# HiLab-git/FPL-plus

Hardware: NVIDIA B200
Metric: train_voxels_per_s (higher is better)
Workload: dtype bf16

## Files before the change

### fpl-plus_b200/build.py

```python
import os
import shutil
import subprocess
import sys

HERE = os.path.dirname(os.path.abspath(__file__))
CSRC = os.path.join(HERE, "csrc")
LIB = os.path.join(HERE, "libfplplus_b200.so")
SOURCES = ["api.cu", "dsbn.cu", "loss.cu", "filter.cu", "conv_direct.cu", "conv_tc.cu", "conv_wgrad_tc.cu", "conv_wgrad_hs.cu", "convt_tc.cu", "conv_tc_dfold.cu", "grad.cu", "adam.cu", "datapath.cu", "head.cu", "head_tc.cu", "stem_tc.cu", "upsample.cu"]
NVCC_FLAGS = ["-gencode", "arch=compute_100a,code=sm_100a", "-lineinfo", "-O3", "-std=c++17",
              "-Xcompiler", "-fPIC", "--use_fast_math=false"]


def _nvcc():
    for cand in (os.environ.get("NVCC"), shutil.which("nvcc"), "/usr/local/cuda/bin/nvcc"):
        if cand and os.path.exists(cand):
            return cand
    raise RuntimeError("nvcc not found; the fplplus_b200 CUDA library cannot be built")


def needs_build():
    if not os.path.exists(LIB):
        return True
    t = os.path.getmtime(LIB)
    deps = [os.path.join(CSRC, f) for f in os.listdir(CSRC)] + [os.path.join(HERE, "..", "include", "fplplus_b200.h")]
# ... 37 lines not shown
```

### fpl-plus_b200/csrc/conv_tc_dfold.cu

```cuda
#include "common.cuh"
#include "tc_ptx.cuh"
#include "../../include/fplplus_b200.h"

namespace {

constexpr int kTileH = 16, kTileW = 8;
constexpr int kBoxH = kTileH + 2, kBoxW = kTileW + 2;
constexpr int kPlaneBytes = kBoxH * kBoxW * 16;
constexpr int kThreadsD = 192;
constexpr int kMaxStagesD = 8;
constexpr int kMaxDC = 16;

struct DfParams {
    const __nv_bfloat16* image;
    const float* bias;
    bf16x8* y;
    int y_c8tot, y_c8off;
    double* stats;
    int N, D, H, W, cin, cout;
    int x_c8tot, x_c8off;
    int nb, nslices, dc, ndc;
    int a_bytes, b_bytes, stages, tmem_cols;
    int pb;
    int tiles_h, tiles_w, total_items;
// ... 480 lines not shown
extern "C" int fpl_conv3d_dfold_prep_weight(const float* w, int cin, int cout, int transpose_flip, void* image, void* stream) {
    return dfold_prep(w, cin, cout, transpose_flip, 9, image, stream);
}

extern "C" int fpl_conv3d_k311_prep_weight(const float* w, int cin, int cout, void* image, void* stream) {
    return dfold_prep(w, cin, cout, 0, 1, image, stream);
}

namespace {
constexpr int kMaxDfBatch = 64;
struct DfPrepBatch {
    const float* w[kMaxDfBatch];
    __nv_bfloat16* image[kMaxDfBatch];
    int cin_eff[kMaxDfBatch], cout_eff[kMaxDfBatch], total[kMaxDfBatch];
    unsigned char tf[kMaxDfBatch], nb[kMaxDfBatch];
};
__global__ void dfold_prep_batch_kernel(const __grid_constant__ DfPrepBatch B) {
    FPL_PDL_WAIT();
    const int e = blockIdx.y;
    const float* __restrict__ w = B.w[e];
    __nv_bfloat16* image = B.image[e];
    const int cin_eff = B.cin_eff[e], cout_eff = B.cout_eff[e], nb = B.nb[e], tf = B.tf[e];
    const int ksteps = cin_eff / 16, n3 = 3 * nb;
    const int pairs = cin_eff * cout_eff;
    for (int r = blockIdx.x * blockDim.x + threadIdx.x; r < pairs; r += gridDim.x * blockDim.x) {
        const int el = r & 7, n = (r >> 3) % nb, jk = (r >> 3) / nb;
        const int in = jk * 8 + el, out = n;
        const float* src = tf ? w + ((int64_t)in * cout_eff + out) * 27 : w + ((int64_t)out * cin_eff + in) * 27;
#pragma unroll
        for (int jj = 0; jj < 3; ++jj) {
#pragma unroll
            for (int t9 = 0; t9 < 9; ++t9) {
                const int tap = (2 - jj) * 9 + t9;
                const float v = __ldg(src + (tf ? 26 - tap : tap));
                image[(((int64_t)t9 * ksteps * 2 + jk) * n3 + jj * nb + n) * 8 + el] = __float2bfloat16_rn(v);
            }
        }
    }
}
}

extern "C" int fpl_conv3d_dfold_prep_weight_batch(int count, const float* const* h_w, const int* h_cin, const int* h_cout,
                                                  const int* h_transpose_flip, void* const* h_images, void* stream) {
    FPL_REQUIRE(count >= 0 && count <= kMaxDfBatch, "fpl_conv3d_dfold_prep_weight_batch: count %d not in [0,%d]", count, kMaxDfBatch);
    if (count == 0) return 0;
    DfPrepBatch B;
    int max_total = 0;
    for (int e = 0; e < count; ++e) {
        const int tf = h_transpose_flip[e];
        const int cin_eff = tf ? h_cout[e] : h_cin[e], cout_eff = tf ? h_cin[e] : h_cout[e];
        DfCfg c;
        FPL_REQUIRE(make_df_cfg(cin_eff, cout_eff, 16, c), "fpl_conv3d_dfold_prep_weight_batch: unsupported channels (%d -> %d)", cin_eff, cout_eff);
        B.w[e] = h_w[e]; B.image[e] = (__nv_bfloat16*)h_images[e]; B.cin_eff[e] = cin_eff; B.cout_eff[e] = cout_eff;
        B.tf[e] = (unsigned char)tf; B.nb[e] = (unsigned char)c.nb; B.total[e] = c.nslices * c.b_bytes / 2;
        if (B.total[e] > max_total) max_total = B.total[e];
    }
    int bx = (max_total / 27 + 255) / 256;
    if (bx > 32) bx = 32;
    if (bx < 1) bx = 1;
    fpl_launch(dfold_prep_batch_kernel, dim3(bx, count), 256, 0, (cudaStream_t)stream, B);
    FPL_LAUNCH_CHECK();
    return 0;
}

static int dfold_launch(const void* x, int x_c8tot, int x_c8off, const void* image, const float* bias, void* y,
                        int y_c8tot, int y_c8off, double* stats, int n, int d, int h, int w, int cin, int cout, int taps,
                        int cin_a, void* stream, const EpiAct* act = nullptr, const EpiBwdRed* br = nullptr) {
    if (cin_a <= 0) cin_a = cin;
    DfCfg c;
    FPL_REQUIRE(make_df_cfg(cin, cout, d, c, taps, cin_a), "fpl_conv3d_tc_dfold: unsupported shape (%d -> %d, depth %d)", cin, cout, d);
    FPL_REQUIRE((reinterpret_cast<uintptr_t>(x) & 15) == 0 && (reinterpret_cast<uintptr_t>(image) & 15) == 0,
                "fpl_conv3d_tc_dfold: x/image must be 16-byte aligned");
    EncodeTiledFn encode = get_encode_fn();
    FPL_REQUIRE(encode != nullptr, "fpl_conv3d_tc_dfold: cuTensorMapEncodeTiled not available from the driver");
    CUtensorMap xmap;
    const int bw = (g_df_tma & 1) ? kTileW : kBoxW, bh = (g_df_tma & 8) ? kTileH : kBoxH;
    const int esz = (g_df_tma & 2) ? 8 : 2;
// ... 91 lines not shown
```

### fpl-plus_b200/lib.py

```python
import ctypes
import os
from ctypes import c_char_p, c_double, c_float, c_int, c_int64, c_longlong, c_uint64, c_void_p

from . import build as _build

_P = c_void_p
_I = c_int
_L = c_int64
_F = c_float
_U = c_uint64

_SIGNATURES = {
    "fpl_last_error": (c_char_p, []),
    "fpl_version": (_I, []),
    "fpl_set_sm_budget": (_I, [_I]),
    "fpl_launch_count": (c_longlong, [_I]),
    "fpl_device_is_sm100": (_I, []),
    "fpl_debug_set": (None, [_I, c_longlong]),
    "fpl_conv3d_weight_image_bytes": (_L, [_I, _I, _I]),
    "fpl_conv3d_prep_weight": (_I, [_P, _I, _I, _I, _I, _P, _P]),
    "fpl_conv3d_prep_weight_batch": (_I, [_I, ctypes.POINTER(c_void_p), ctypes.POINTER(_I), ctypes.POINTER(_I),
                                          ctypes.POINTER(_I), ctypes.POINTER(_I), ctypes.POINTER(c_void_p), _P]),
    "fpl_conv3d_tc": (_I, [_P, _I, _I, _P, _P, _P, _I, _I, _P] + [_I] * 7 + [_P]),
    "fpl_conv3d_dfold_image_bytes": (_L, [_I, _I]),
    "fpl_conv3d_dfold_prep_weight": (_I, [_P, _I, _I, _I, _P, _P]),
    "fpl_conv3d_dfold_prep_weight_batch": (_I, [_I, ctypes.POINTER(c_void_p), ctypes.POINTER(_I), ctypes.POINTER(_I),
                                                ctypes.POINTER(_I), ctypes.POINTER(c_void_p), _P]),
    "fpl_conv3d_tc_dfold": (_I, [_P, _I, _I, _P, _P, _P, _I, _I, _P] + [_I] * 6 + [_P]),
    "fpl_patch9_c8": (_I, [_P, _P, _I, _I, _I, _I, _I, _P]),
    "fpl_conv3d_k311_prep_weight": (_I, [_P, _I, _I, _P, _P]),
    "fpl_conv3d_tc_k311": (_I, [_P, _I, _I, _P, _P, _P, _I, _I, _P] + [_I] * 7 + [_P]),
    "fpl_conv3d_wgrad_tc_k311": (_I, [_P, _I, _I, _P, _I, _I, _P] + [_I] * 6 + [_P]),
    "fpl_conv3d_direct": (_I, [_P, _I, _I, _P, _P, _P, _I, _I, _P] + [_I] * 9 + [_P]),
    "fpl_conv3d_wgrad": (_I, [_P, _I, _I, _P, _I, _I, _P] + [_I] * 7 + [_P]),
    "fpl_conv3d_wgrad_tc": (_I, [_P, _I, _I, _P, _I, _I, _P] + [_I] * 7 + [_P]),
    "fpl_conv3d_wgrad_tc_tapmajor": (_I, [_P, _I, _I, _P, _I, _I, _P] + [_I] * 7 + [_P]),
    "fpl_wgrad_tapmajor_to_dw_batch": (_I, [_I, ctypes.POINTER(c_void_p), ctypes.POINTER(c_void_p), ctypes.POINTER(_I),
                                            ctypes.POINTER(_I), ctypes.POINTER(_I), ctypes.POINTER(_I), _P]),
    "fpl_dsbn_eval_affine_batch": (_I, [_I] + [ctypes.POINTER(c_void_p)] * 7 + [ctypes.POINTER(_I), _F, _P]),
    "fpl_conv3d_tc_act": (_I, [_P, _I, _I, _P, _P, _I, _I] + [_I] * 7 + [_P, _P, _P, _F, _U, _U, _P, _P]),
    "fpl_conv3d_tc_dfold_act": (_I, [_P, _I, _I, _P, _P, _I, _I] + [_I] * 6 + [_P, _P, _P, _P]),
    "fpl_conv3d_tc_k311_act": (_I, [_P, _I, _I, _P, _P, _I, _I] + [_I] * 7 + [_P, _P, _P, _P]),
    "fpl_maxpool_c8": (_I, [_P, _I, _I, _P, _I, _I, _I] + [_I] * 5 + [_P]),
    "fpl_head_fwd": (_I, [_P, _I, _I, _P, _P, _P] + [_I] * 6 + [_P]),
    "fpl_head_dgrad": (_I, [_P, _P, _P, _I, _I, _P, _I, _I, _P] + [_I] * 6 + [_P]),
    "fpl_upsample2x_c8": (_I, [_P, _I, _I, _P, _I, _I] + [_I] * 6 + [_P]),
    "fpl_upsample2x_c8_bwd": (_I, [_P, _I, _I, _P, _I, _I] + [_I] * 6 + [_P]),
    "fpl_channel_sum_c8": (_I, [_P, _I, _I, _P] + [_I] * 5 + [_P]),
    "fpl_grad_scatter_add": (_I, [_P, _P, _P, _I, _I, _P]),
    "fpl_stem_conv_fwd": (_I, [_P, _P, _P, _P, _I, _I, _P] + [_I] * 7 + [_P]),
    "fpl_stem_conv_wgrad": (_I, [_P, _P, _I, _I, _P] + [_I] * 7 + [_P]),
    "fpl_head_conv_fwd": (_I, [_P, _I, _I, _P, _P, _P] + [_I] * 6 + [_P]),
    "fpl_head_conv_tc": (_I, [_P, _I, _I, _P, _P, _P] + [_I] * 6 + [_P]),
    "fpl_pack_ncdhw_to_c8": (_I, [_P, _I, _P, _I, _I, _I, _P] + [_I] * 4 + [_P]),
    "fpl_head_conv_bwd": (_I, [_P, _I, _I, _P, _P, _P, _I, _I, _P, _P] + [_I] * 6 + [_P]),
    "fpl_convt_k2s2_fwd": (_I, [_P, _I, _I, _P, _P, _P, _I, _I] + [_I] * 7 + [_P]),
# ... 94 lines not shown
```

### fpl-plus_b200/net.py

```python
import ctypes
import os

import torch
import torch.nn as nn

from . import ops
from .ops import C8, call, ptr, stream_ptr


class DomainSpecificBatchNorm2d(nn.Module):
    def __init__(self, num_features, num_domains):
        super().__init__()
        self.bns = nn.ModuleList([nn.BatchNorm2d(num_features) for _ in range(num_domains)])


class DomainSpecificBatchNorm3d(nn.Module):
    def __init__(self, num_features, num_domains):
        super().__init__()
        self.bns = nn.ModuleList([nn.BatchNorm3d(num_features) for _ in range(num_domains)])


class ConvBlockND(nn.Module):

    def __init__(self, in_channels, out_channels, num_domains=None, dim=2, dropout_p=0.5):
# ... 108 lines not shown
        self._infer_ws = None
        self._img_cache = {}
        self._dropout_masks = None
        self._rng_dev = None
        self._rng_lanes = {}
        self._cur_lane = 0
        self._seed_from_device = False
        self._graphs = {}
        self._graph_ws_keep = []
        self._infer_wss = {}
        self.cuda_graphs = os.environ.get("FPL_CUDA_GRAPH", "1") != "0"
        self.wgrad_side_stream = os.environ.get("FPL_WGRAD_STREAM", "0") != "0"
        self._aux_streams = {}
        self._dfold_cache = {}
        self._unit_depth = {}
        self.grad_ready_hook = None
        self.grad_wait_hook = None
        self.grad_bucket_bytes = 4 << 20
        self.grad_tail_bytes = 3 << 19
        self._master = None
        self._head = UNet2D5_dsbn._HeadConv(self.out_conv)
        self._stem = None
        self._head_unit = None
        self._head_dirty = True
        self._stem_dirty = True
        self._geo0 = (0, 0, 0)
        self._grad_pass = False
        self._build_plan()

    def _build_plan(self):
# ... 268 lines not shown

    def _refresh_weight_images(self, with_dgrad):
        lib = ops._lib.load()
        if self._stem_tc(self._unit_depth.get("block0.conv#1", 0)) and not (with_dgrad and self._stem_direct(self._geo0)):
            if self._stem is None:
                self._stem = UNet2D5_dsbn._StemConv(self._down_units[0][0].conv)
            self._stem.sync(self._stem_dirty)
            self._stem_dirty = False
        todo, todo_df, todo_ct = [], [], []
        for u in self._tc_convs():
            w = u.conv.weight
            depth = self._unit_depth.get(u.name, 0)
            for transpose in ((False, True) if with_dgrad else (False,)):
                if transpose and not self._use_tc(u.cout, u.cin):
                    continue
                if u.name != "head" and self._dfold_ok(u.cout if transpose else u.cin, u.cin if transpose else u.cout,
                                                       u.kd, depth):
                    if not (transpose and u.name == "block0.conv#1"):
                        self._dfold_image(u.conv, transpose, todo_df)
                    continue
                key = (id(w), transpose)
                ent = self._img_cache.get(key)
                if ent is None or ent[1].device != w.device:
                    nbytes = lib.fpl_conv3d_weight_image_bytes(u.cout if transpose else u.cin,
                                                               u.cin if transpose else u.cout, u.kd)
                    ent = self._img_cache[key] = [-1, torch.empty(nbytes // 2, dtype=torch.bfloat16, device=w.device)]
                if ent[0] != w._version:
                    todo.append((w, u.cin, u.cout, u.kd, 1 if transpose else 0, ent))
        if os.environ.get("FPL_CONVT_IMPL", "tc") == "tc":
            for up in (self.up1, self.up2, self.up3, self.up4):
                trans = up.trans3d if up.dim == 3 else up.trans2d
                if self._use_tc(trans.weight.shape[0], trans.weight.shape[1]):
                    kd2 = 2 if up.dim == 3 else 1
                    self._convt_image(trans, kd2, 0, todo_ct)
                    if with_dgrad:
                        self._convt_image(trans, kd2, 1, todo_ct)
        for i in range(0, len(todo_df), 64):
            part = todo_df[i:i + 64]
            n = len(part)
            arr_w = (ctypes.c_void_p * n)(*[t[0].data_ptr() for t in part])
            arr_img = (ctypes.c_void_p * n)(*[t[4][1].data_ptr() for t in part])
            ints = [(ctypes.c_int * n)(*[t[k] for t in part]) for k in (1, 2, 3)]
            call("fpl_conv3d_dfold_prep_weight_batch", n, arr_w, ints[0], ints[1], ints[2], arr_img, stream_ptr())
            for t in part:
                t[4][0] = t[0]._version
        if todo_ct:
            n = len(todo_ct)
            arr_w = (ctypes.c_void_p * n)(*[t[0].data_ptr() for t in todo_ct])
            arr_img = (ctypes.c_void_p * n)(*[t[5][1].data_ptr() for t in todo_ct])
            ints = [(ctypes.c_int * n)(*[t[k] for t in todo_ct]) for k in (1, 2, 3, 4)]
            call("fpl_convt_prep_weight_batch", n, arr_w, ints[0], ints[1], ints[2], ints[3], arr_img, stream_ptr())
            for t in todo_ct:
                t[5][0] = t[0]._version
        for i in range(0, len(todo), 80):
            part = todo[i:i + 80]
            n = len(part)
            arr_w = (ctypes.c_void_p * n)(*[t[0].data_ptr() for t in part])
            arr_img = (ctypes.c_void_p * n)(*[t[5][1].data_ptr() for t in part])
            ints = [(ctypes.c_int * n)(*[t[k] for t in part]) for k in (1, 2, 3, 4)]
            call("fpl_conv3d_prep_weight_batch", n, arr_w, ints[0], ints[1], ints[2], ints[3], arr_img, stream_ptr())
            for t in part:
                t[5][0] = t[0]._version

    def _note_depths(self, geo):
        self._geo0 = tuple(geo[0])
        for i in range(5):
            for u in self._down_units[i]:
                self._unit_depth[u.name] = geo[i][0]
        for k, lvl in zip(range(4), (3, 2, 1, 0)):
            for u in self._up_units[k]:
                self._unit_depth[u.name] = geo[lvl][0]

    def _dfold_ok(self, cin, cout, kd, depth):
        if kd != 3 or depth < 2 or not self._use_tc(cin, cout) or os.environ.get("FPL_DFOLD", "1") == "0":
            return False
        key = (cin, cout)
        ok = self._dfold_cache.get(key)
        if ok is None:
            ok = self._dfold_cache[key] = ops._lib.load().fpl_conv3d_dfold_image_bytes(cin, cout) > 0
        return ok

    def _dfold_image(self, conv, transpose, defer=None):
        w = conv.weight
        key = (id(w), "df%d" % (1 if transpose else 0))
        ent = self._img_cache.get(key)
        cin, cout = conv.in_channels, conv.out_channels
        if ent is None or ent[1].device != w.device:
            nbytes = ops._lib.load().fpl_conv3d_dfold_image_bytes(cout if transpose else cin, cin if transpose else cout)
            ent = self._img_cache[key] = [-1, torch.empty(nbytes // 2, dtype=torch.bfloat16, device=w.device)]
        if ent[0] != w._version:
            if defer is not None:
                defer.append((w, cin, cout, 1 if transpose else 0, ent))
            else:
                call("fpl_conv3d_dfold_prep_weight", ptr(w), cin, cout, 1 if transpose else 0, ptr(ent[1]), stream_ptr())
                ent[0] = w._version
        return ent[1]

    def _convt_tc(self, cin, cout):
        return (self._use_tc(cin, cout) and os.environ.get("FPL_CONVT_IMPL", "tc") == "tc")

    def _convt_image(self, trans, kd2, mode, defer=None):
        w = trans.weight
        key = (id(w), "ct%d" % mode)
        ent = self._img_cache.get(key)
        if ent is None or ent[1].device != w.device:
            nbytes = ops._lib.load().fpl_convt_weight_image_bytes(w.shape[0], w.shape[1], kd2)
            ent = self._img_cache[key] = [-1, torch.empty(nbytes // 2, dtype=torch.bfloat16, device=w.device)]
        if ent[0] != w._version:
            if defer is not None:
# ... 9 lines not shown
            self._refresh_weight_images(with_dgrad=transpose)
            ent = self._img_cache[(id(conv.weight), transpose)]
        return ent[1]

    def _conv_fwd(self, u, xin, x_img, y, stats, n, geo, ws):
        d, h, w = geo
        st = stream_ptr()
        if u.is_stem and self._stem_tc(d) and not (self._grad_pass and self._stem_direct(geo)):
            xs = ws.c8("XS:stem", n, d, 32, h, w)
            call("fpl_patch9_c8", ptr(x_img), ptr(xs), 1, n, d, h, w, st)
            call("fpl_conv3d_tc_k311", ptr(xs), 4, 0, ptr(self._stem.image), ptr(u.conv.bias), ptr(y), y.shape[2], 0,
                 ptr(stats), n, d, h, w, 48, u.cout, 32, st)
        elif u.is_stem:
            call("fpl_stem_conv_fwd", ptr(x_img), ptr(u.conv.weight), ptr(u.conv.bias), ptr(y), y.shape[2], 0,
                 ptr(stats), n, u.cin, d, h, w, u.cout, u.kd, st)
        elif self._dfold_ok(u.cin, u.cout, u.kd, d):
            call("fpl_conv3d_tc_dfold", *xin.args(), ptr(self._dfold_image(u.conv, False)), ptr(u.conv.bias), ptr(y),
                 y.shape[2], 0, ptr(stats), n, d, h, w, u.cin, u.cout, st)
        elif self._use_tc(u.cin, u.cout):
            img = self._weight_image(u.conv, u.kd, False, ws)
            call("fpl_conv3d_tc", *xin.args(), ptr(img), ptr(u.conv.bias), ptr(y), y.shape[2], 0, ptr(stats),
                 n, d, h, w, u.cin, u.cout, u.kd, st)
        else:
            call("fpl_conv3d_direct", *xin.args(), ptr(u.conv.weight), ptr(u.conv.bias), ptr(y), y.shape[2], 0,
                 ptr(stats), n, d, h, w, u.cin, u.cout, u.kd, 0, 0, st)

    def _eval_affine_refresh(self, domain, ws):
        units = [u for pair in self._down_units + self._up_units for u in pair if not u.dsbn.bns[domain].training]
        if not units or os.environ.get("FPL_EVAL_FUSE", "1") == "0" or not ops.is_sm100():
            return {}
# ... 16 lines not shown
    def _unit_fwd_fused(self, u, xin, x_img, out, aff, p, seed, offset, seed_dev, n, geo, ws):
        d, h, w = geo
        st = stream_ptr()
        scale, shift = aff
        if u.is_stem:
            if not self._stem_tc(d) or p > 0.0:
                return False
            xs = ws.c8("XS:stem", n, d, 32, h, w)
            call("fpl_patch9_c8", ptr(x_img), ptr(xs), 1, n, d, h, w, st)
            call("fpl_conv3d_tc_k311_act", ptr(xs), 4, 0, ptr(self._stem.image), *out.args(), n, d, h, w, 48, u.cout, 32,
                 ptr(scale), ptr(shift), ptr(u.prelu.weight), st)
            return True
        if self._dfold_ok(u.cin, u.cout, u.kd, d):
            if p > 0.0:
                return False
            call("fpl_conv3d_tc_dfold_act", *xin.args(), ptr(self._dfold_image(u.conv, False)), *out.args(), n, d, h, w,
                 u.cin, u.cout, ptr(scale), ptr(shift), ptr(u.prelu.weight), st)
            return True
        if self._use_tc(u.cin, u.cout):
            img = self._weight_image(u.conv, u.kd, False, ws)
            call("fpl_conv3d_tc_act", *xin.args(), ptr(img), *out.args(), n, d, h, w, u.cin, u.cout, u.kd, ptr(scale),
                 ptr(shift), ptr(u.prelu.weight), p, seed, offset, ptr(seed_dev) if p > 0.0 else None, st)
            return True
        return False

    def _unit_fwd(self, u, domain, xin, x_img, out, pooled, pool_idx, pool_kd, n, geo, ws, small, rec):
        d, h, w = geo
        c = u.cout
        aff = rec["eval_affine"].get(u.name)
        if aff is not None:
# ... 201 lines not shown
        else:
            self._wgrad(u, xin, dy, dw, n, d, h, w, fold)
        if not need_dx:
            return None
        dx = ws.c8("dX:" + u.name, n, d, u.cin, h, w)
        br = None
        if prev is not None and self._bwdred_ok(*prev) and (self._dfold_ok(u.cout, u.cin, u.kd, d) or self._use_tc(u.cout, u.cin)):
            up, rp = prev
            rp["red_fused"] = small.f64(2 * up.cout + 1)
            br = (ptr(rp["y"]), ptr(rp["scale"]), ptr(rp["shift"]), ptr(rp["mean"]), ptr(rp["invstd"]), ptr(up.prelu.weight),
                  rp["p"], rp["seed"], rp["offset"], ptr(rp["seed_dev"]), ptr(rp["red_fused"]))
        if self._dfold_ok(u.cout, u.cin, u.kd, d):
            if br is not None:
                call("fpl_conv3d_tc_dfold_bwdred", ptr(dy), c // 8, 0, ptr(self._dfold_image(u.conv, True)), ptr(dx),
                     u.cin // 8, 0, n, d, h, w, c, u.cin, *br, st)
            else:
                call("fpl_conv3d_tc_dfold", ptr(dy), c // 8, 0, ptr(self._dfold_image(u.conv, True)), None, ptr(dx),
                     u.cin // 8, 0, None, n, d, h, w, c, u.cin, st)
        elif self._use_tc(u.cout, u.cin):
            img = self._weight_image(u.conv, u.kd, True, ws)
            if br is not None:
                call("fpl_conv3d_tc_bwdred", ptr(dy), c // 8, 0, ptr(img), ptr(dx), u.cin // 8, 0, n, d, h, w, c, u.cin,
                     u.kd, *br, st)
            else:
                call("fpl_conv3d_tc", ptr(dy), c // 8, 0, ptr(img), None, ptr(dx), u.cin // 8, 0, None,
                     n, d, h, w, c, u.cin, u.kd, st)
        else:
            call("fpl_conv3d_direct", ptr(dy), c // 8, 0, ptr(u.conv.weight), None, ptr(dx), u.cin // 8, 0, None,
                 n, d, h, w, c, u.cin, u.kd, 1, 0, st)
        return C8(dx)
# ... 310 lines not shown
```

### include/fplplus_b200.h

```cpp
#ifndef FPLPLUS_B200_H
#define FPLPLUS_B200_H

#include <stdint.h>

#ifdef __cplusplus
extern "C" {
#endif

const char* fpl_last_error(void);
int fpl_version(void);
int fpl_set_sm_budget(int sms);
long long fpl_launch_count(int reset);
int fpl_device_is_sm100(void);
void fpl_debug_set(int key, long long value);


int64_t fpl_conv3d_weight_image_bytes(int cin, int cout, int kd);
int fpl_conv3d_prep_weight(const float* w, int cin, int cout, int kd, int transpose_flip,
                           void* image, void* stream);
int fpl_conv3d_prep_weight_batch(int count, const float* const* h_w, const int* h_cin, const int* h_cout,
                                 const int* h_kd, const int* h_transpose_flip, void* const* h_images, void* stream);
int fpl_conv3d_tc(const void* x, int x_c8tot, int x_c8off, const void* image, const float* bias,
                  void* y, int y_c8tot, int y_c8off, double* stats,
                  int n, int d, int h, int w, int cin, int cout, int kd, void* stream);
int64_t fpl_conv3d_dfold_image_bytes(int cin, int cout);
int fpl_conv3d_dfold_prep_weight(const float* w, int cin, int cout, int transpose_flip, void* image, void* stream);
int fpl_conv3d_dfold_prep_weight_batch(int count, const float* const* h_w, const int* h_cin, const int* h_cout,
                                       const int* h_transpose_flip, void* const* h_images, void* stream);
int fpl_conv3d_tc_dfold(const void* x, int x_c8tot, int x_c8off, const void* image, const float* bias,
                        void* y, int y_c8tot, int y_c8off, double* stats,
                        int n, int d, int h, int w, int cin, int cout, void* stream);
int fpl_patch9_c8(const float* x, void* out, int split_hi_lo, int n, int d, int h, int w, void* stream);
int fpl_conv3d_k311_prep_weight(const float* w, int cin, int cout, void* image, void* stream);
int fpl_conv3d_tc_k311(const void* x, int x_c8tot, int x_c8off, const void* image, const float* bias,
                       void* y, int y_c8tot, int y_c8off, double* stats,
                       int n, int d, int h, int w, int cin, int cout, int a_channels, void* stream);
int fpl_conv3d_wgrad_tc_k311(const void* x, int x_c8tot, int x_c8off, const void* dy, int dy_c8tot, int dy_c8off,
                             float* dw, int n, int d, int h, int w, int cin, int cout, void* stream);
int fpl_conv3d_direct(const void* x, int x_c8tot, int x_c8off, const float* w, const float* bias,
                      void* y, int y_c8tot, int y_c8off, double* stats,
                      int n, int d, int h, int w_, int cin, int cout, int kd,
                      int transpose_flip, int round_w_bf16, void* stream);
int fpl_conv3d_wgrad(const void* x, int x_c8tot, int x_c8off, const void* dy, int dy_c8tot, int dy_c8off,
                     float* dw, int n, int d, int h, int w, int cin, int cout, int kd, void* stream);

int fpl_conv3d_wgrad_tc(const void* x, int x_c8tot, int x_c8off, const void* dy, int dy_c8tot, int dy_c8off,
// ... 24 lines not shown
                          double lr_host, double beta1, double beta2, double eps, double weight_decay,
                          unsigned int* d_done_counter, void* stream);
int fpl_adam_chunk_elems(void);

int fpl_dsbn_eval_affine_batch(int count, const float* const* h_gamma, const float* const* h_beta,
                               const float* const* h_running_mean, const float* const* h_running_var,
                               const float* const* h_conv_bias, float* const* h_scale, float* const* h_shift,
                               const int* h_c, float eps, void* stream);
int fpl_conv3d_tc_act(const void* x, int x_c8tot, int x_c8off, const void* image, void* a, int a_c8tot, int a_c8off,
                      int n, int d, int h, int w, int cin, int cout, int kd, const float* scale, const float* shift,
                      const float* slope, float drop_p, uint64_t seed, uint64_t offset, const uint64_t* seed_dev,
                      void* stream);
int fpl_conv3d_tc_dfold_act(const void* x, int x_c8tot, int x_c8off, const void* image, void* a, int a_c8tot, int a_c8off,
                            int n, int d, int h, int w, int cin, int cout, const float* scale, const float* shift,
                            const float* slope, void* stream);
int fpl_conv3d_tc_k311_act(const void* x, int x_c8tot, int x_c8off, const void* image, void* a, int a_c8tot, int a_c8off,
                           int n, int d, int h, int w, int cin, int cout, int a_channels, const float* scale,
                           const float* shift, const float* slope, void* stream);

int fpl_maxpool_c8(const void* a, int a_c8tot, int a_c8off, void* pooled, int p_c8tot, int p_c8off, int pool_kd,
                   int n, int d, int h, int w, int c, void* stream);

int fpl_head_fwd(const void* x, int x_c8tot, int x_c8off, const float* w, const float* bias, float* logits, int n, int d,
                 int h, int w_, int cin, int classes, void* stream);
int fpl_head_dgrad(const float* dlogits, const float* w, void* g, int g_c8tot, int g_c8off, void* dl8, int dl_c8tot,
                   int dl_c8off, float* dbias, int n, int d, int h, int w_, int cin, int classes, void* stream);

int fpl_upsample2x_c8(const void* x, int x_c8tot, int x_c8off, void* y, int y_c8tot, int y_c8off, int n, int d, int h, int w,
                      int c, int kd2, void* stream);
int fpl_upsample2x_c8_bwd(const void* gy, int gy_c8tot, int gy_c8off, void* gx, int gx_c8tot, int gx_c8off, int n, int d,
// ... 118 lines not shown
```

Before: 1.003 billion.

## Add row-column tensor-core conv kernel for 16-channel full-width layers

Adds a new tcgen05 3D conv kernel for the 16/32→16-channel layers at width 128. Each unit is one full image row over a chunk of depth slices. It loads whole rows by TMA, reuses the H-neighbour rows across consecutive units, and folds the W taps into the MMA N dimension. Horizontal neighbours are combined in the epilogue through warp shuffles and a small shared exchange buffer. The aim is to cut halo reloads and tile overhead compared with the 16x8 dfold tiling, at the cost of extra weight images, a separate prep path and a more complex epilogue. It is wired into forward, the fused act path and backward dgrad.

Result: slower. 837.3 million (median of 6 runs) (-16.5%).

```diff
diff --git a/fpl-plus_b200/build.py b/fpl-plus_b200/build.py
--- a/fpl-plus_b200/build.py
+++ b/fpl-plus_b200/build.py
@@ -6,7 +6,7 @@
 HERE = os.path.dirname(os.path.abspath(__file__))
 CSRC = os.path.join(HERE, "csrc")
 LIB = os.path.join(HERE, "libfplplus_b200.so")
-SOURCES = ["api.cu", "dsbn.cu", "loss.cu", "filter.cu", "conv_direct.cu", "conv_tc.cu", "conv_wgrad_tc.cu", "conv_wgrad_hs.cu", "convt_tc.cu", "conv_tc_dfold.cu", "grad.cu", "adam.cu", "datapath.cu", "head.cu", "head_tc.cu", "stem_tc.cu", "upsample.cu"]
+SOURCES = ["api.cu", "dsbn.cu", "loss.cu", "filter.cu", "conv_direct.cu", "conv_tc.cu", "conv_wgrad_tc.cu", "conv_wgrad_hs.cu", "convt_tc.cu", "conv_tc_dfold.cu", "conv_tc_coln.cu", "grad.cu", "adam.cu", "datapath.cu", "head.cu", "head_tc.cu", "stem_tc.cu", "upsample.cu"]
 NVCC_FLAGS = ["-gencode", "arch=compute_100a,code=sm_100a", "-lineinfo", "-O3", "-std=c++17",
               "-Xcompiler", "-fPIC", "--use_fast_math=false"]
 
diff --git a/fpl-plus_b200/csrc/conv_tc_coln.cu b/fpl-plus_b200/csrc/conv_tc_coln.cu
--- /dev/null
+++ b/fpl-plus_b200/csrc/conv_tc_coln.cu
@@ -0,0 +1,345 @@
+#include "common.cuh"
+#include "tc_ptx.cuh"
+#include "../../include/fplplus_b200.h"
+
+namespace {
+
+constexpr int kCnW = 128;
+constexpr int kCnRowBytes = kCnW * 16;
+#ifndef FPL_COLN_DC
+#define FPL_COLN_DC 4
+#endif
+#ifndef FPL_COLN_STAGES
+#define FPL_COLN_STAGES 8
+#endif
+constexpr int kCnDC = FPL_COLN_DC;
+constexpr int kCnPB = kCnDC + 2;
+constexpr int kCnN = 144;
+constexpr int kCnCols = kCnDC * 48;
+constexpr uint32_t kCnTmemCols = 2 * kCnCols <= 256 ? 256u : 512u;
+constexpr int kCnEpiWarps = 8;
+constexpr int kCnThreads = 64 + 32 * kCnEpiWarps;
+constexpr int kCnMaxStages = 8;
+constexpr int kCnSmemMax = 227 * 1024;
+
+struct CnParams {
+    const __nv_bfloat16* image;
+    const float* bias;
+    bf16x8* y;
+    int y_c8tot, y_c8off;
+    double* stats;
+    int N, D, H, cin;
+    int x_c8off;
+    int nchunks, units;
+    int a_bytes, b_bytes, stages;
+    EpiAct act;
+};
+
+__device__ __forceinline__ void cn_tmem_st_zero16(uint32_t taddr) {
+    const uint32_t z = 0u;
+    asm volatile(
+        "tcgen05.st.sync.aligned.32x32b.x16.b32 [%0], {%1,%1,%1,%1,%1,%1,%1,%1,%1,%1,%1,%1,%1,%1,%1,%1};"
+        ::"r"(taddr), "r"(z) : "memory");
+}
+__device__ __forceinline__ void cn_tmem_st_wait() { asm volatile("tcgen05.wait::st.sync.aligned;" ::: "memory"); }
+__device__ __forceinline__ void cn_bar_sync(int id, int threads) { asm volatile("bar.sync %0, %1;" ::"r"(id), "r"(threads) : "memory"); }
+
+struct CnUnit {
+    int n, d0, dcount, h;
+};
+__device__ __forceinline__ CnUnit cn_unit(const CnParams& P, int u) {
+    CnUnit c;
+    const int col = u / P.H;
+    c.h = u - col * P.H;
+    const int ch = col % P.nchunks;
+    c.n = col / P.nchunks;
+    c.d0 = ch * kCnDC;
+    c.dcount = min(kCnDC, P.D - c.d0);
+    return c;
+}
+
+template <int KSTEPS>
+__global__ void __launch_bounds__(kCnThreads, 1) conv3d_tc_coln_kernel(const __grid_constant__ CUtensorMap xmap, CnParams P) {
+    extern __shared__ uint8_t smem_raw[];
+    uint8_t* smem = reinterpret_cast<uint8_t*>((reinterpret_cast<uintptr_t>(smem_raw) + 1023) & ~uintptr_t(1023));
+    uint8_t* b_sm = smem;
+    uint8_t* ring = smem + ((P.b_bytes + 1023) & ~1023);
+    uint64_t* bars = reinterpret_cast<uint64_t*>(ring + (size_t)P.stages * P.a_bytes);
+    uint64_t* full_bar = bars;
+    uint64_t* empty_bar = bars + kCnMaxStages;
+    uint64_t* acc_full = bars + 2 * kCnMaxStages;
+    uint64_t* acc_empty = acc_full + 2;
+    uint64_t* w_bar = acc_empty + 2;
+    uint32_t* tmem_slot = reinterpret_cast<uint32_t*>(w_bar + 1);
+    float* xch = reinterpret_cast<float*>(bars + 2 * kCnMaxStages + 8);
+    float* bias_sm = xch + 2 * 2 * 4 * 2 * 16;
+    float* scale_sm = bias_sm + 16;
+
+    const int warp = threadIdx.x >> 5, lane = threadIdx.x & 31;
+    const int u_begin = (int)(((int64_t)blockIdx.x * P.units) / gridDim.x);
+    const int u_end = (int)(((int64_t)(blockIdx.x + 1) * P.units) / gridDim.x);
+    if (warp == 0 && lane == 0) {
+        asm volatile("prefetch.tensormap [%0];" ::"l"(&xmap) : "memory");
+        for (int s = 0; s < P.stages; ++s) { mbar_init(&full_bar[s], 1); mbar_init(&empty_bar[s], 1); }
+        for (int a = 0; a < 2; ++a) { mbar_init(&acc_full[a], 1); mbar_init(&acc_empty[a], kCnEpiWarps); }
+        mbar_init(w_bar, 1);
+        fence_barrier_init();
+    }
+    if (warp == 1) tmem_alloc(tmem_slot, kCnTmemCols);
+    FPL_PDL_WAIT();
+    const bool fuse_act = P.act.scale != nullptr;
+    if (threadIdx.x < 16) {
+        bias_sm[threadIdx.x] = fuse_act ? P.act.shift[threadIdx.x] : (P.bias != nullptr ? P.bias[threadIdx.x] : 0.0f);
+        scale_sm[threadIdx.x] = fuse_act ? P.act.scale[threadIdx.x] : 1.0f;
+    }
+    tc_fence_before();
+    __syncthreads();
+    tc_fence_after();
+    const uint32_t tmem_base = *tmem_slot;
+
+    if (warp == 0) {
+        if (lane == 0) {
+            mbar_expect_tx(w_bar, (uint32_t)P.b_bytes);
+            bulk_load(b_sm, P.image, (uint32_t)P.b_bytes, w_bar);
+            int stage = 0; uint32_t phase = 0;
+            for (int u = u_begin; u < u_end; ++u) {
+                const CnUnit c = cn_unit(P, u);
+                const int first = (u == u_begin || c.h == 0) ? c.h - 1 : c.h + 1;
+                for (int r = first; r <= c.h + 1; ++r) {
+                    mbar_wait(&empty_bar[stage], phase ^ 1);
+                    mbar_expect_tx(&full_bar[stage], (uint32_t)P.a_bytes);
+                    tma_load_5d(ring + (size_t)stage * P.a_bytes, &xmap, &full_bar[stage], 0, r, P.x_c8off, c.d0 - 1, c.n);
+                    if (++stage == P.stages) { stage = 0; phase ^= 1; }
+                }
+            }
+        }
+    } else if (warp == 1) {
+        const uint32_t idesc0 = (1u << 4) | (1u << 7) | (1u << 10) | (8u << 24);
+        const uint64_t a_hi = make_desc(0, kCnRowBytes, 128);
+        const uint64_t b0 = make_desc(0, kCnN * 16, 128) + (uint64_t)(smem_u32(b_sm) >> 4);
+        const uint32_t ring_u = smem_u32(ring) >> 4;
+        constexpr int c8 = 2 * KSTEPS;
+        const uint32_t a_stage = (uint32_t)P.a_bytes >> 4;
+        const uint64_t b_kstep = (uint64_t)(2 * kCnN);
+        const bool leader = elect_one();
+        int q_next = 0;
+        uint32_t acc_phase = 0u;
+        mbar_wait(w_bar, 0);
+        for (int u = u_begin; u < u_end; ++u) {
+            const CnUnit c = cn_unit(P, u);
+            if (u == u_begin || c.h == 0) q_next += 2;
+            const int q0 = q_next - 2;
+            ++q_next;
+            const int a = u & 1;
+            mbar_wait(&acc_empty[a], (acc_phase >> a) & 1u);
+            acc_phase ^= 1u << a;
+            uint32_t st_base[3];
+#pragma unroll
+            for (int k = 0; k < 3; ++k) {
+                const int q = q0 + k, s = q % P.stages;
+                mbar_wait(&full_bar[s], (uint32_t)(q / P.stages) & 1u);
+                st_base[k] = ring_u + (uint32_t)s * a_stage;
+            }
+            tc_fence_after();
+            const uint32_t d_set = tmem_base + (uint32_t)(a * kCnCols);
+            for (int i = 0; i < kCnPB; ++i) {
+                const int z = c.d0 - 1 + i;
+                const int jlo = i < 2 ? 2 - i : 0;
+                const int jhi = min(2, c.dcount + 1 - i);
+                if (z < 0 || z >= P.D || jlo > jhi) continue;
+                const uint32_t ncols = (uint32_t)(jhi - jlo + 1) * 48u;
+                const uint32_t idesc = idesc0 | ((ncols >> 3) << 17);
+                const uint32_t d_tmem = d_set + (uint32_t)((i - 2 + jlo) * 48);
+                const uint64_t bj = b0 + (uint64_t)(jlo * 48);
+                if (leader) {
+#pragma unroll
+                    for (int kh = 0; kh < 3; ++kh) {
+                        const uint64_t ak = a_hi + (uint64_t)(st_base[kh] + (uint32_t)(i * c8) * (kCnRowBytes / 16));
+                        const uint64_t bk = bj + (uint64_t)(kh * KSTEPS) * b_kstep;
+#pragma unroll
+                        for (int j = 0; j < KSTEPS; ++j)
+                            umma_bf16(d_tmem, ak + (uint64_t)(j * 2 * (kCnRowBytes / 16)), bk + (uint64_t)j * b_kstep, idesc, 1u);
+                    }
+                }
+                __syncwarp();
+            }
+            if (leader) {
+                umma_commit(&acc_full[a]);
+                umma_commit(&empty_bar[q0 % P.stages]);
+                if (u + 1 == u_end || c.h + 1 == P.H) {
+                    umma_commit(&empty_bar[(q0 + 1) % P.stages]);
+                    umma_commit(&empty_bar[(q0 + 2) % P.stages]);
+                }
+            }
+            __syncwarp();
+        }
+        FPL_PDL_TRIGGER();
+    } else {
+        const int quarter = warp & 3, pair = (warp - 2) >> 2;
+        const int w = quarter * 32 + lane;
+        const uint32_t lane_base = tmem_base + ((uint32_t)(quarter * 32) << 16);
+        const bool want_stats = P.stats != nullptr;
+        const float act_slope = fuse_act ? __ldg(P.act.slope) : 0.0f;
+        float tacc[32];
+#pragma unroll
+        for (int i = 0; i < 32; ++i) tacc[i] = 0.0f;
+        for (int col = 0; col < kCnCols; col += 16) cn_tmem_st_zero16(lane_base + (uint32_t)(pair * kCnCols + col));
+        cn_tmem_st_wait();
+        tc_fence_before();
+        __syncwarp();
+        if (lane == 0) { mbar_arrive(&acc_empty[0]); mbar_arrive(&acc_empty[1]); }
+        const int64_t HW = (int64_t)P.H * kCnW;
+        uint32_t acc_phase = 0u;
+        int it = 0;
+        for (int u = u_begin; u < u_end; ++u) {
+            const CnUnit c = cn_unit(P, u);
+            const int a = u & 1;
+            mbar_wait(&acc_full[a], (acc_phase >> a) & 1u);
+            acc_phase ^= 1u << a;
+            tc_fence_after();
+            for (int p = pair; p < c.dcount; p += 2, ++it) {
+                const uint32_t taddr = lane_base + (uint32_t)(a * kCnCols + p * 48);
+                uint32_t r0[16], r1[16], r2[16];
+                tmem_ld16(taddr, r0);
+                tmem_ld16(taddr + 16, r1);
+                tmem_ld16(taddr + 32, r2);
+                tmem_ld_wait();
+                cn_tmem_st_zero16(taddr);
+                cn_tmem_st_zero16(taddr + 16);
+                cn_tmem_st_zero16(taddr + 32);
+                float* xb = xch + ((it & 1) * 2 + pair) * 4 * 32;
+                if (lane == 31) {
+#pragma unroll
+                    for (int i = 0; i < 16; ++i) xb[quarter * 32 + i] = __uint_as_float(r0[i]);
+                }
+                if (lane == 0) {
+#pragma unroll
+                    for (int i = 0; i < 16; ++i) xb[quarter * 32 + 16 + i] = __uint_as_float(r2[i]);
+                }
+                cn_bar_sync(1 + pair, 128);
+                float v[16];
+#pragma unroll
+                for (int i = 0; i < 16; ++i) {
+                    float left = __shfl_up_sync(0xffffffffu, __uint_as_float(r0[i]), 1);
+                    float right = __shfl_down_sync(0xffffffffu, __uint_as_float(r2[i]), 1);
+                    if (lane == 0) left = quarter > 0 ? xb[(quarter - 1) * 32 + i] : 0.0f;
+                    if (lane == 31) right = quarter < 3 ? xb[(quarter + 1) * 32 + 16 + i] : 0.0f;
+                    const float acc = left + __uint_as_float(r1[i]) + right;
+                    if (!fuse_act) {
+                        v[i] = acc + bias_sm[i];
+                    } else {
+                        const float zz = fmaf(acc, scale_sm[i], bias_sm[i]);
+                        v[i] = zz > 0.0f ? zz : act_slope * zz;
+                    }
+                }
+                const int64_t out = (((int64_t)c.n * P.D + c.d0 + p) * P.y_c8tot + P.y_c8off) * HW + (int64_t)c.h * kCnW + w;
+                st_bf16x8(P.y + out, v);
+                st_bf16x8(P.y + out + HW, v + 8);
+                if (want_stats) {
+#pragma unroll
+                    for (int i = 0; i < 16; ++i) {
+                        tacc[i] += v[i];
+                        tacc[16 + i] = fmaf(v[i], v[i], tacc[16 + i]);
+                    }
+                }
+            }
+            cn_tmem_st_wait();
+            tc_fence_before();
+            __syncwarp();
+            if (lane == 0) mbar_arrive(&acc_empty[a]);
+        }
+        if (want_stats && u_begin < u_end) {
+            warp_transpose_sum32(tacc, lane);
+            atomicAdd(P.stats + (lane >> 4) * 16 + (lane & 15), (double)tacc[0]);
+        }
+    }
+    tc_fence_before();
+    __syncthreads();
+    if (warp == 1) {
+        tc_fence_after();
+        tmem_dealloc(tmem_base, kCnTmemCols);
+    }
+}
+
+struct CnCfg {
+    int a_bytes, b_bytes, stages, smem_bytes;
+};
+
+bool make_cn_cfg(int cin, int cout, int w, CnCfg& c) {
+    if (cout != 16 || (cin != 16 && cin != 32) || w != kCnW) return false;
+    c.b_bytes = 27 * cin * 16 * 2;
+    c.a_bytes = (cin / 8) * kCnPB * kCnRowBytes;
+    const int fixed = ((c.b_bytes + 1023) & ~1023) + 1024 + (2 * kCnMaxStages + 8) * 8 + (2 * 2 * 4 * 2 * 16 + 32) * 4;
+    c.stages = (kCnSmemMax - fixed) / c.a_bytes;
+    if (c.stages > FPL_COLN_STAGES) c.stages = FPL_COLN_STAGES;
+    if (c.stages < 4) return false;
+    c.smem_bytes = fixed + c.stages * c.a_bytes;
+    return true;
+}
+
+}
+
+extern "C" int fpl_conv3d_coln_supported(int cin, int cout, int w) {
+    CnCfg c;
+    return make_cn_cfg(cin, cout, w, c) ? 1 : 0;
+}
+
+static int coln_launch(const void* x, int x_c8tot, int x_c8off, const void* image, const float* bias, void* y, int y_c8tot,
+                       int y_c8off, double* stats, int n, int d, int h, int w, int cin, int cout, void* stream,
+                       const EpiAct* act) {
+    CnCfg c;
+    FPL_REQUIRE(make_cn_cfg(cin, cout, w, c), "fpl_conv3d_tc_coln: unsupported shape (%d -> %d, W %d): needs Cin 16 / 32, Cout 16, W 128",
+                cin, cout, w);
+    FPL_REQUIRE(n >= 1 && d >= 1 && h >= 1, "fpl_conv3d_tc_coln: empty volume (%d x %d x %d x %d)", n, d, h, w);
+    FPL_REQUIRE(x_c8off >= 0 && x_c8off + cin / 8 <= x_c8tot && y_c8off >= 0 && y_c8off + 2 <= y_c8tot,
+                "fpl_conv3d_tc_coln: channel slice out of range");
+    FPL_REQUIRE((reinterpret_cast<uintptr_t>(x) & 15) == 0 && (reinterpret_cast<uintptr_t>(image) & 15) == 0 &&
+                (reinterpret_cast<uintptr_t>(y) & 15) == 0, "fpl_conv3d_tc_coln: x/image/y must be 16-byte aligned");
+    EncodeTiledFn encode = get_encode_fn();
+    FPL_REQUIRE(encode != nullptr, "fpl_conv3d_tc_coln: cuTensorMapEncodeTiled not available from the driver");
+    CUtensorMap xmap;
+    cuuint64_t gdim[5] = {(cuuint64_t)w * 2, (cuuint64_t)h, (cuuint64_t)x_c8tot, (cuuint64_t)d, (cuuint64_t)n};
+    cuuint64_t gstride[4] = {(cuuint64_t)w * 16, (cuuint64_t)h * w * 16, (cuuint64_t)x_c8tot * h * w * 16,
+                             (cuuint64_t)d * x_c8tot * h * w * 16};
+    cuuint32_t box[5] = {(cuuint32_t)kCnW * 2, 1, (cuuint32_t)(cin / 8), (cuuint32_t)kCnPB, 1};
+    cuuint32_t estr[5] = {1, 1, 1, 1, 1};
+    CUresult r = encode(&xmap, CU_TENSOR_MAP_DATA_TYPE_UINT64, 5, const_cast<void*>(x), gdim, gstride, box, estr,
+                        CU_TENSOR_MAP_INTERLEAVE_NONE, CU_TENSOR_MAP_SWIZZLE_NONE, CU_TENSOR_MAP_L2_PROMOTION_L2_256B,
+                        CU_TENSOR_MAP_FLOAT_OOB_FILL_NONE);
+    FPL_REQUIRE(r == CUDA_SUCCESS, "fpl_conv3d_tc_coln: cuTensorMapEncodeTiled failed (%d)", (int)r);
+    CnParams P;
+    P.image = (const __nv_bfloat16*)image; P.bias = bias; P.y = (bf16x8*)y; P.y_c8tot = y_c8tot; P.y_c8off = y_c8off;
+    P.stats = stats; P.N = n; P.D = d; P.H = h; P.cin = cin; P.x_c8off = x_c8off;
+    P.nchunks = (d + kCnDC - 1) / kCnDC;
+    const int64_t units = (int64_t)n * P.nchunks * h;
+    FPL_REQUIRE(units < (1ll << 30), "fpl_conv3d_tc_coln: too many rows");
+    P.units = (int)units;
+    P.a_bytes = c.a_bytes; P.b_bytes = c.b_bytes; P.stages = c.stages;
+    if (act != nullptr) P.act = *act; else { P.act.scale = nullptr; P.act.shift = nullptr; P.act.slope = nullptr; P.act.drop_p = 0.0f; P.act.seed = P.act.offset = 0; P.act.seed_dev = nullptr; }
+    int grid = FPL_NUM_SMS;
+    if (grid > P.units) grid = P.units;
+    if (cin == 16) {
+        FPL_CHECK_CUDA(cudaFuncSetAttribute(conv3d_tc_coln_kernel<1>, cudaFuncAttributeMaxDynamicSharedMemorySize, c.smem_bytes));
+        fpl_launch(conv3d_tc_coln_kernel<1>, grid, kCnThreads, c.smem_bytes, (cudaStream_t)stream, xmap, P);
+    } else {
+        FPL_CHECK_CUDA(cudaFuncSetAttribute(conv3d_tc_coln_kernel<2>, cudaFuncAttributeMaxDynamicSharedMemorySize, c.smem_bytes));
+        fpl_launch(conv3d_tc_coln_kernel<2>, grid, kCnThreads, c.smem_bytes, (cudaStream_t)stream, xmap, P);
+    }
+    FPL_LAUNCH_CHECK();
+    return 0;
+}
+
+extern "C" int fpl_conv3d_tc_coln(const void* x, int x_c8tot, int x_c8off, const void* image, const float* bias, void* y,
+                                  int y_c8tot, int y_c8off, double* stats, int n, int d, int h, int w, int cin, int cout,
+                                  void* stream) {
+    return coln_launch(x, x_c8tot, x_c8off, image, bias, y, y_c8tot, y_c8off, stats, n, d, h, w, cin, cout, stream, nullptr);
+}
+
+extern "C" int fpl_conv3d_tc_coln_act(const void* x, int x_c8tot, int x_c8off, const void* image, void* a, int a_c8tot,
+                                      int a_c8off, int n, int d, int h, int w, int cin, int cout, const float* scale,
+                                      const float* shift, const float* slope, void* stream) {
+    FPL_REQUIRE(scale != nullptr && shift != nullptr && slope != nullptr, "fpl_conv3d_tc_coln_act: scale/shift/slope required");
+    EpiAct act;
+    act.scale = scale; act.shift = shift; act.slope = slope; act.drop_p = 0.0f; act.seed = act.offset = 0; act.seed_dev = nullptr;
+    return coln_launch(x, x_c8tot, x_c8off, image, nullptr, a, a_c8tot, a_c8off, nullptr, n, d, h, w, cin, cout, stream, &act);
+}
diff --git a/fpl-plus_b200/csrc/conv_tc_dfold.cu b/fpl-plus_b200/csrc/conv_tc_dfold.cu
--- a/fpl-plus_b200/csrc/conv_tc_dfold.cu
+++ b/fpl-plus_b200/csrc/conv_tc_dfold.cu
@@ -518,13 +518,14 @@
     __nv_bfloat16* image[kMaxDfBatch];
     int cin_eff[kMaxDfBatch], cout_eff[kMaxDfBatch], total[kMaxDfBatch];
     unsigned char tf[kMaxDfBatch], nb[kMaxDfBatch];
+    unsigned char coln[kMaxDfBatch];
 };
 __global__ void dfold_prep_batch_kernel(const __grid_constant__ DfPrepBatch B) {
     FPL_PDL_WAIT();
     const int e = blockIdx.y;
     const float* __restrict__ w = B.w[e];
     __nv_bfloat16* image = B.image[e];
-    const int cin_eff = B.cin_eff[e], cout_eff = B.cout_eff[e], nb = B.nb[e], tf = B.tf[e];
+    const int cin_eff = B.cin_eff[e], cout_eff = B.cout_eff[e], nb = B.nb[e], tf = B.tf[e], coln = B.coln[e];
     const int ksteps = cin_eff / 16, n3 = 3 * nb;
     const int pairs = cin_eff * cout_eff;
     for (int r = blockIdx.x * blockDim.x + threadIdx.x; r < pairs; r += gridDim.x * blockDim.x) {
@@ -537,7 +538,9 @@
             for (int t9 = 0; t9 < 9; ++t9) {
                 const int tap = (2 - jj) * 9 + t9;
                 const float v = __ldg(src + (tf ? 26 - tap : tap));
-                image[(((int64_t)t9 * ksteps * 2 + jk) * n3 + jj * nb + n) * 8 + el] = __float2bfloat16_rn(v);
+                const int64_t pos = coln ? (((int64_t)(t9 / 3) * ksteps * 2 + jk) * 144 + jj * 48 + (t9 % 3) * 16 + n) * 8 + el
+                                         : (((int64_t)t9 * ksteps * 2 + jk) * n3 + jj * nb + n) * 8 + el;
+                image[pos] = __float2bfloat16_rn(v);
             }
         }
     }
@@ -545,7 +548,8 @@
 }
 
 extern "C" int fpl_conv3d_dfold_prep_weight_batch(int count, const float* const* h_w, const int* h_cin, const int* h_cout,
-                                                  const int* h_transpose_flip, void* const* h_images, void* stream) {
+                                                  const int* h_transpose_flip, const int* h_coln, void* const* h_images,
+                                                  void* stream) {
     FPL_REQUIRE(count >= 0 && count <= kMaxDfBatch, "fpl_conv3d_dfold_prep_weight_batch: count %d not in [0,%d]", count, kMaxDfBatch);
     if (count == 0) return 0;
     DfPrepBatch B;
@@ -556,7 +560,11 @@
         DfCfg c;
         FPL_REQUIRE(make_df_cfg(cin_eff, cout_eff, 16, c), "fpl_conv3d_dfold_prep_weight_batch: unsupported channels (%d -> %d)", cin_eff, cout_eff);
         B.w[e] = h_w[e]; B.image[e] = (__nv_bfloat16*)h_images[e]; B.cin_eff[e] = cin_eff; B.cout_eff[e] = cout_eff;
+        const int coln = h_coln != nullptr && h_coln[e] != 0;
+        FPL_REQUIRE(!coln || (cout_eff == 16 && (cin_eff == 16 || cin_eff == 32)),
+                    "fpl_conv3d_dfold_prep_weight_batch: no column-tap layout for %d -> %d", cin_eff, cout_eff);
         B.tf[e] = (unsigned char)tf; B.nb[e] = (unsigned char)c.nb; B.total[e] = c.nslices * c.b_bytes / 2;
+        B.coln[e] = (unsigned char)coln;
         if (B.total[e] > max_total) max_total = B.total[e];
     }
     int bx = (max_total / 27 + 255) / 256;
@@ -565,6 +573,11 @@
     fpl_launch(dfold_prep_batch_kernel, dim3(bx, count), 256, 0, (cudaStream_t)stream, B);
     FPL_LAUNCH_CHECK();
     return 0;
+}
+
+extern "C" int fpl_conv3d_coln_prep_weight(const float* w, int cin, int cout, int transpose_flip, void* image, void* stream) {
+    const int coln = 1;
+    return fpl_conv3d_dfold_prep_weight_batch(1, &w, &cin, &cout, &transpose_flip, &coln, &image, stream);
 }
 
 static int dfold_launch(const void* x, int x_c8tot, int x_c8off, const void* image, const float* bias, void* y,
diff --git a/fpl-plus_b200/lib.py b/fpl-plus_b200/lib.py
--- a/fpl-plus_b200/lib.py
+++ b/fpl-plus_b200/lib.py
@@ -25,8 +25,11 @@
     "fpl_conv3d_dfold_image_bytes": (_L, [_I, _I]),
     "fpl_conv3d_dfold_prep_weight": (_I, [_P, _I, _I, _I, _P, _P]),
     "fpl_conv3d_dfold_prep_weight_batch": (_I, [_I, ctypes.POINTER(c_void_p), ctypes.POINTER(_I), ctypes.POINTER(_I),
-                                                ctypes.POINTER(_I), ctypes.POINTER(c_void_p), _P]),
+                                                ctypes.POINTER(_I), ctypes.POINTER(_I), ctypes.POINTER(c_void_p), _P]),
     "fpl_conv3d_tc_dfold": (_I, [_P, _I, _I, _P, _P, _P, _I, _I, _P] + [_I] * 6 + [_P]),
+    "fpl_conv3d_coln_supported": (_I, [_I, _I, _I]),
+    "fpl_conv3d_coln_prep_weight": (_I, [_P, _I, _I, _I, _P, _P]),
+    "fpl_conv3d_tc_coln": (_I, [_P, _I, _I, _P, _P, _P, _I, _I, _P] + [_I] * 6 + [_P]),
     "fpl_patch9_c8": (_I, [_P, _P, _I, _I, _I, _I, _I, _P]),
     "fpl_conv3d_k311_prep_weight": (_I, [_P, _I, _I, _P, _P]),
     "fpl_conv3d_tc_k311": (_I, [_P, _I, _I, _P, _P, _P, _I, _I, _P] + [_I] * 7 + [_P]),
@@ -40,6 +43,7 @@
     "fpl_dsbn_eval_affine_batch": (_I, [_I] + [ctypes.POINTER(c_void_p)] * 7 + [ctypes.POINTER(_I), _F, _P]),
     "fpl_conv3d_tc_act": (_I, [_P, _I, _I, _P, _P, _I, _I] + [_I] * 7 + [_P, _P, _P, _F, _U, _U, _P, _P]),
     "fpl_conv3d_tc_dfold_act": (_I, [_P, _I, _I, _P, _P, _I, _I] + [_I] * 6 + [_P, _P, _P, _P]),
+    "fpl_conv3d_tc_coln_act": (_I, [_P, _I, _I, _P, _P, _I, _I] + [_I] * 6 + [_P, _P, _P, _P]),
     "fpl_conv3d_tc_k311_act": (_I, [_P, _I, _I, _P, _P, _I, _I] + [_I] * 7 + [_P, _P, _P, _P]),
     "fpl_maxpool_c8": (_I, [_P, _I, _I, _P, _I, _I, _I] + [_I] * 5 + [_P]),
     "fpl_head_fwd": (_I, [_P, _I, _I, _P, _P, _P] + [_I] * 6 + [_P]),
diff --git a/fpl-plus_b200/net.py b/fpl-plus_b200/net.py
--- a/fpl-plus_b200/net.py
+++ b/fpl-plus_b200/net.py
@@ -146,6 +146,8 @@
         self._aux_streams = {}
         self._dfold_cache = {}
         self._unit_depth = {}
+        self._unit_width = {}
+        self._coln_cache = {}
         self.grad_ready_hook = None
         self.grad_wait_hook = None
         self.grad_bucket_bytes = 4 << 20
@@ -444,10 +446,14 @@
             for transpose in ((False, True) if with_dgrad else (False,)):
                 if transpose and not self._use_tc(u.cout, u.cin):
                     continue
-                if u.name != "head" and self._dfold_ok(u.cout if transpose else u.cin, u.cin if transpose else u.cout,
-                                                       u.kd, depth):
+                ci, co = (u.cout, u.cin) if transpose else (u.cin, u.cout)
+                if u.name != "head" and self._dfold_ok(ci, co, u.kd, depth):
                     if not (transpose and u.name == "block0.conv#1"):
-                        self._dfold_image(u.conv, transpose, todo_df)
+                        coln = self._coln_ok(ci, co, u.kd, self._unit_width.get(u.name, 0))
+                        if coln:
+                            self._dfold_image(u.conv, transpose, todo_df, coln=True)
+                        if not coln or (transpose and os.environ.get("FPL_BWD_FUSE", "0") != "0"):
+                            self._dfold_image(u.conv, transpose, todo_df)
                     continue
                 key = (id(w), transpose)
                 ent = self._img_cache.get(key)
@@ -470,8 +476,8 @@
             n = len(part)
             arr_w = (ctypes.c_void_p * n)(*[t[0].data_ptr() for t in part])
             arr_img = (ctypes.c_void_p * n)(*[t[4][1].data_ptr() for t in part])
-            ints = [(ctypes.c_int * n)(*[t[k] for t in part]) for k in (1, 2, 3)]
-            call("fpl_conv3d_dfold_prep_weight_batch", n, arr_w, ints[0], ints[1], ints[2], arr_img, stream_ptr())
+            ints = [(ctypes.c_int * n)(*[t[k] for t in part]) for k in (1, 2, 3, 5)]
+            call("fpl_conv3d_dfold_prep_weight_batch", n, arr_w, ints[0], ints[1], ints[2], ints[3], arr_img, stream_ptr())
             for t in part:
                 t[4][0] = t[0]._version
         if todo_ct:
@@ -497,9 +503,11 @@
         for i in range(5):
             for u in self._down_units[i]:
                 self._unit_depth[u.name] = geo[i][0]
+                self._unit_width[u.name] = geo[i][2]
         for k, lvl in zip(range(4), (3, 2, 1, 0)):
             for u in self._up_units[k]:
                 self._unit_depth[u.name] = geo[lvl][0]
+                self._unit_width[u.name] = geo[lvl][2]
 
     def _dfold_ok(self, cin, cout, kd, depth):
         if kd != 3 or depth < 2 or not self._use_tc(cin, cout) or os.environ.get("FPL_DFOLD", "1") == "0":
@@ -510,9 +518,18 @@
             ok = self._dfold_cache[key] = ops._lib.load().fpl_conv3d_dfold_image_bytes(cin, cout) > 0
         return ok
 
-    def _dfold_image(self, conv, transpose, defer=None):
+    def _coln_ok(self, cin, cout, kd, width):
+        if not self._dfold_ok(cin, cout, kd, 2):
+            return False
+        key = (cin, cout, width)
+        ok = self._coln_cache.get(key)
+        if ok is None:
+            ok = self._coln_cache[key] = bool(ops._lib.load().fpl_conv3d_coln_supported(cin, cout, width))
+        return ok
+
+    def _dfold_image(self, conv, transpose, defer=None, coln=False):
         w = conv.weight
-        key = (id(w), "df%d" % (1 if transpose else 0))
+        key = (id(w), "%s%d" % ("cn" if coln else "df", 1 if transpose else 0))
         ent = self._img_cache.get(key)
         cin, cout = conv.in_channels, conv.out_channels
         if ent is None or ent[1].device != w.device:
@@ -520,9 +537,10 @@
             ent = self._img_cache[key] = [-1, torch.empty(nbytes // 2, dtype=torch.bfloat16, device=w.device)]
         if ent[0] != w._version:
             if defer is not None:
-                defer.append((w, cin, cout, 1 if transpose else 0, ent))
-            else:
-                call("fpl_conv3d_dfold_prep_weight", ptr(w), cin, cout, 1 if transpose else 0, ptr(ent[1]), stream_ptr())
+                defer.append((w, cin, cout, 1 if transpose else 0, ent, 1 if coln else 0))
+            else:
+                call("fpl_conv3d_coln_prep_weight" if coln else "fpl_conv3d_dfold_prep_weight", ptr(w), cin, cout,
+                     1 if transpose else 0, ptr(ent[1]), stream_ptr())
                 ent[0] = w._version
         return ent[1]
 
@@ -562,6 +580,9 @@
         elif u.is_stem:
             call("fpl_stem_conv_fwd", ptr(x_img), ptr(u.conv.weight), ptr(u.conv.bias), ptr(y), y.shape[2], 0,
                  ptr(stats), n, u.cin, d, h, w, u.cout, u.kd, st)
+        elif self._coln_ok(u.cin, u.cout, u.kd, w) and d >= 2:
+            call("fpl_conv3d_tc_coln", *xin.args(), ptr(self._dfold_image(u.conv, False, coln=True)), ptr(u.conv.bias),
+                 ptr(y), y.shape[2], 0, ptr(stats), n, d, h, w, u.cin, u.cout, st)
         elif self._dfold_ok(u.cin, u.cout, u.kd, d):
             call("fpl_conv3d_tc_dfold", *xin.args(), ptr(self._dfold_image(u.conv, False)), ptr(u.conv.bias), ptr(y),
                  y.shape[2], 0, ptr(stats), n, d, h, w, u.cin, u.cout, st)
@@ -608,6 +629,10 @@
         if self._dfold_ok(u.cin, u.cout, u.kd, d):
             if p > 0.0:
                 return False
+            if self._coln_ok(u.cin, u.cout, u.kd, w):
+                call("fpl_conv3d_tc_coln_act", *xin.args(), ptr(self._dfold_image(u.conv, False, coln=True)), *out.args(),
+                     n, d, h, w, u.cin, u.cout, ptr(scale), ptr(shift), ptr(u.prelu.weight), st)
+                return True
             call("fpl_conv3d_tc_dfold_act", *xin.args(), ptr(self._dfold_image(u.conv, False)), *out.args(), n, d, h, w,
                  u.cin, u.cout, ptr(scale), ptr(shift), ptr(u.prelu.weight), st)
             return True
@@ -839,6 +864,9 @@
             if br is not None:
                 call("fpl_conv3d_tc_dfold_bwdred", ptr(dy), c // 8, 0, ptr(self._dfold_image(u.conv, True)), ptr(dx),
                      u.cin // 8, 0, n, d, h, w, c, u.cin, *br, st)
+            elif self._coln_ok(u.cout, u.cin, u.kd, w):
+                call("fpl_conv3d_tc_coln", ptr(dy), c // 8, 0, ptr(self._dfold_image(u.conv, True, coln=True)), None,
+                     ptr(dx), u.cin // 8, 0, None, n, d, h, w, c, u.cin, st)
             else:
                 call("fpl_conv3d_tc_dfold", ptr(dy), c // 8, 0, ptr(self._dfold_image(u.conv, True)), None, ptr(dx),
                      u.cin // 8, 0, None, n, d, h, w, c, u.cin, st)
diff --git a/include/fplplus_b200.h b/include/fplplus_b200.h
--- a/include/fplplus_b200.h
+++ b/include/fplplus_b200.h
@@ -26,10 +26,16 @@
 int64_t fpl_conv3d_dfold_image_bytes(int cin, int cout);
 int fpl_conv3d_dfold_prep_weight(const float* w, int cin, int cout, int transpose_flip, void* image, void* stream);
 int fpl_conv3d_dfold_prep_weight_batch(int count, const float* const* h_w, const int* h_cin, const int* h_cout,
-                                       const int* h_transpose_flip, void* const* h_images, void* stream);
+                                       const int* h_transpose_flip, const int* h_coln, void* const* h_images,
+                                       void* stream);
 int fpl_conv3d_tc_dfold(const void* x, int x_c8tot, int x_c8off, const void* image, const float* bias,
                         void* y, int y_c8tot, int y_c8off, double* stats,
                         int n, int d, int h, int w, int cin, int cout, void* stream);
+int fpl_conv3d_coln_supported(int cin, int cout, int w);
+int fpl_conv3d_coln_prep_weight(const float* w, int cin, int cout, int transpose_flip, void* image, void* stream);
+int fpl_conv3d_tc_coln(const void* x, int x_c8tot, int x_c8off, const void* image, const float* bias,
+                       void* y, int y_c8tot, int y_c8off, double* stats,
+                       int n, int d, int h, int w, int cin, int cout, void* stream);
 int fpl_patch9_c8(const float* x, void* out, int split_hi_lo, int n, int d, int h, int w, void* stream);
 int fpl_conv3d_k311_prep_weight(const float* w, int cin, int cout, void* image, void* stream);
 int fpl_conv3d_tc_k311(const void* x, int x_c8tot, int x_c8off, const void* image, const float* bias,
@@ -84,6 +90,9 @@
 int fpl_conv3d_tc_dfold_act(const void* x, int x_c8tot, int x_c8off, const void* image, void* a, int a_c8tot, int a_c8off,
                             int n, int d, int h, int w, int cin, int cout, const float* scale, const float* shift,
                             const float* slope, void* stream);
+int fpl_conv3d_tc_coln_act(const void* x, int x_c8tot, int x_c8off, const void* image, void* a, int a_c8tot, int a_c8off,
+                           int n, int d, int h, int w, int cin, int cout, const float* scale, const float* shift,
+                           const float* slope, void* stream);
 int fpl_conv3d_tc_k311_act(const void* x, int x_c8tot, int x_c8off, const void* image, void* a, int a_c8tot, int a_c8off,
                            int n, int d, int h, int w, int cin, int cout, int a_channels, const float* scale,
                            const float* shift, const float* slope, void* stream);
```
